# danieleschmidt/spin-glass-anneal-rl

Measured on AMD Instinct MI355X. Metric: spin-flip attempts/s (replicas x spins x sweeps / s), higher is better.
Workload: dtype f32

## Files before the change

spin-glass-anneal-rl_amd/csrc/sweep_dense_rs.hip:

```cpp
#include <cstdio>
#include <cstring>
#include <type_traits>

#include "sweep_common.h"

namespace sga {

template <bool GRID>
using RsPlanArg = typename std::conditional<GRID, RowSharedGridPlan, RowSharedPlan>::type;
__device__ __forceinline__ const RowSharedPlan &rs_plan(const RowSharedPlan &p) { return p; }
__device__ __forceinline__ const RowSharedPlan &rs_plan(const RowSharedGridPlan &g) { return g.p; }
__device__ __forceinline__ int rs_grid_k(const RowSharedPlan &) { return 0; }
__device__ __forceinline__ int rs_grid_k(const RowSharedGridPlan &g) { return g.k; }

__device__ __forceinline__ void rs_bit_of(int j, int &w32, unsigned int &bit) {
    const int g = j >> 8, e = j & 255, l = e >> 2, q = e & 3;
    w32 = 2 * (4 * g + q) + (l >> 5);
    bit = 1u << (l & 31);
}

__device__ __forceinline__ void rs_update(const SweepArgs &a, int r, int k, int t, int &site, uint32_t &ubits) {
    const u32x4 w = philox4x32_10((uint32_t)(t >> 1), a.sweep0 + (uint32_t)k, a.replica0 + (uint32_t)r, DOMAIN_SWEEP,
                                  a.seed_lo, a.seed_hi);
    const bool second = t & 1;
// ... 186 lines not shown
    for (int j = 0; j < NP; ++j) {
        const int x = tid + j * T, rr = x >> lhalf, b = x & hmask;
#pragma unroll
        for (int h = 0; h < 2; ++h) {
            const int s = site[2 * j + h];
            if (s < 0) continue;
            int ls;
            const int tl = rs_tile_of(s, S, mul, ls) - tl0;
            stage[atomicAdd(&cnt[(tl << log_trg) + rr], 1)] = ls | (rr << 12) | ((2 * b + h) << 17);
        }
    }
    __syncthreads();
    int *dst = p.ent + (long long)a.R * t0 + (long long)r0 * nt + below;
    for (int i = tid, m = sums[1]; i < m; i += T) dst[i] = stage[i];
}

template <typename JE, int PL, bool GRID>
__device__ __forceinline__ int rs_row_to_planes(const JE *row, int n, unsigned long long *planes, int lane, int wv, int gk) {
    const int nseg = (n + 255) >> 8, nw = 4 * nseg;
    int absum = 0;
    for (int g0 = wv; g0 < nseg; g0 += 16) {
        int v[4][4];
#pragma unroll
        for (int s = 0; s < 4; ++s) {
            const int e = 256 * (g0 + 4 * s) + 4 * lane;
            if (g0 + 4 * s < nseg && e < n) {
                if constexpr (std::is_same<JE, float>::value) {
                    float4 x = *reinterpret_cast<const float4 *>(row + e);
                    if constexpr (GRID) x.x = ldexpf(x.x, gk), x.y = ldexpf(x.y, gk), x.z = ldexpf(x.z, gk), x.w = ldexpf(x.w, gk);
                    v[s][0] = (int)x.x, v[s][1] = (int)x.y, v[s][2] = (int)x.z, v[s][3] = (int)x.w;
                } else {
                    const int x = *reinterpret_cast<const int *>(row + e);
#pragma unroll
                    for (int q = 0; q < 4; ++q) v[s][q] = (int)(int8_t)(x >> (8 * q));
                }
            } else {
#pragma unroll
                for (int q = 0; q < 4; ++q) v[s][q] = 0;
            }
#pragma unroll
            for (int q = 0; q < 4; ++q)
                if (e + q >= n) v[s][q] = 0;
        }
#pragma unroll
        for (int s = 0; s < 4; ++s) {
            const int g = g0 + 4 * s;
            if (g >= nseg) break;
#pragma unroll
            for (int q = 0; q < 4; ++q) {
                const int m = v[s][q] < 0 ? -v[s][q] : v[s][q];
                absum += m;
                const unsigned long long sg = ballot64(v[s][q] < 0);
                unsigned long long pb[PL];
#pragma unroll
                for (int b = 0; b < PL; ++b) pb[b] = ballot64(((m >> b) & 1) != 0);
                if (lane == 0) {
                    planes[4 * g + q] = sg;
#pragma unroll
                    for (int b = 0; b < PL; ++b) planes[(long long)(1 + b) * nw + 4 * g + q] = pb[b];
                }
            }
        }
    }
    return absum;
}

template <typename JE, int PL>
__global__ void __launch_bounds__(256) rs_planes_kernel(const JE *J, long long ldj, int n, unsigned long long *jp, int *jabs) {
    __shared__ int csum[4];
    const int i = blockIdx.x, lane = threadIdx.x & 63, wv = threadIdx.x >> 6;
    const int nw = 4 * ((n + 255) >> 8);
    int absum = rs_row_to_planes<JE, PL, false>(J + (long long)i * ldj, n, jp + (long long)i * (PL + 1) * nw, lane, wv, 0);
    absum = wave_sum(absum);
    if (lane == 0) csum[wv] = absum;
    __syncthreads();
    if (threadIdx.x == 0) jabs[i] = csum[0] + csum[1] + csum[2] + csum[3];
}
template <int PL>
__global__ void __launch_bounds__(256) rs_planes_grid_kernel(const float *J, long long ldj, int n, unsigned long long *jp, int *jabs,
                                                             int gk) {
    __shared__ int csum[4];
    const int i = blockIdx.x, lane = threadIdx.x & 63, wv = threadIdx.x >> 6;
    const int nw = 4 * ((n + 255) >> 8);
    int absum = rs_row_to_planes<float, PL, true>(J + (long long)i * ldj, n, jp + (long long)i * (PL + 1) * nw, lane, wv, gk);
    absum = wave_sum(absum);
    if (lane == 0) csum[wv] = absum;
    __syncthreads();
    if (threadIdx.x == 0) jabs[i] = csum[0] + csum[1] + csum[2] + csum[3];
}

template <int PL>
__global__ void __launch_bounds__(256) rs_fields_planes_kernel(const SweepArgs a, RowSharedPlan p, int win) {
    const int i = blockIdx.x, n = a.n;
    const int *off = p.off + (long long)win * (n + 1);
    const int lo = off[i], hi = off[i + 1];
    if (lo == hi) return;
    extern __shared__ ulonglong2 prow[];
    const int nw2 = p.nw32 >> 2;
    const int tid = threadIdx.x, lane = tid & 63, wv = tid >> 6, sub = lane >> 4, l16 = lane & 15;
    const ulonglong2 *src = reinterpret_cast<const ulonglong2 *>(p.jp) + (long long)i * (PL + 1) * nw2;
    for (int c = tid; c < (PL + 1) * nw2; c += 256) prow[c] = src[c];
    const int C = p.jabs[i];
    __syncthreads();
    const ulonglong2 *bits = reinterpret_cast<const ulonglong2 *>(p.bits);
    const int wmask = (1 << p.log_w) - 1;
    for (int x0 = lo + 4 * wv; x0 < hi; x0 += 16) {
        const int x = x0 + sub;
        const bool live = x < hi;
        const int e = p.ent[live ? x : lo];
        const ulonglong2 *s = bits + (long long)(e >> p.log_w) * nw2;
        int acc = 0;
        for (int c = l16; c < nw2; c += 16) {
            const ulonglong2 sv = s[c], sg = prow[c];
            const unsigned long long x0w = sv.x ^ sg.x, x1w = sv.y ^ sg.y;
#pragma unroll
            for (int b = 0; b < PL; ++b) {
                const ulonglong2 pb = prow[(1 + b) * nw2 + c];
                acc += (__popcll(pb.x & x0w) + __popcll(pb.y & x1w)) << b;
            }
        }
        acc += dpp_move<DPP_QUAD_XOR1>(acc);
        acc += dpp_move<DPP_QUAD_XOR2>(acc);
        acc += dpp_move<DPP_ROW_HALF_MIRROR>(acc);
        acc += dpp_move<DPP_ROW_MIRROR>(acc);
        if (live && l16 == 0) p.base[(long long)(e >> p.log_w) * p.W + (e & wmask)] = C - 2 * acc;
    }
}

template <int PL, bool ONES>
__device__ __forceinline__ int rs_tile_word(const ulonglong2 sv, const ulonglong2 *row, int nw2, int c) {
    const ulonglong2 sg = row[c];
    const unsigned long long x0w = sv.x ^ sg.x, x1w = sv.y ^ sg.y;
    if constexpr (ONES) {
        return __popcll(x0w) + __popcll(x1w);
    } else {
        int acc = 0;
#pragma unroll
        for (int b = 0; b < PL; ++b) {
            const ulonglong2 pb = row[(1 + b) * nw2 + c];
            acc += (__popcll(pb.x & x0w) + __popcll(pb.y & x1w)) << b;
        }
        return acc;
    }
}

struct RsTileChunk {
    const int *sent;
    const unsigned short *sls;
    const int *sjabs;
    const ulonglong2 *prow, *bits;
    int *base;
    int cn, nw2, rw2, log_w, W, nwaves;
};
template <int PL, bool ONES, int NK>
__device__ __forceinline__ void rs_tile_pieces(const RsTileChunk &ch, int wv, int sub, int l16) {
    const int L = (ch.cn + 4 * ch.nwaves - 1) / (4 * ch.nwaves), x1 = (4 * wv + sub) * L, wmask = (1 << ch.log_w) - 1;
    constexpr int NR = NK > 0 ? NK : 1;
    const int clast = l16 + 16 * (NR - 1);
    const bool vlast = clast < ch.nw2;
    const int cl = vlast ? clast : 0;
    ulonglong2 sv[NR];
#pragma unroll
    for (int k = 0; k < NR; ++k) sv[k] = make_ulonglong2(0ull, 0ull);
    int rcur = -1;
    for (int t = 0; t < L; ++t) {
        const int x = x1 + t;
        const bool live = x < ch.cn;
        const int e = ch.sent[live ? x : 0], lsd = ch.sls[live ? x : 0], ls = lsd & 0x7fff, r = e >> ch.log_w;
        const ulonglong2 *s = ch.bits + (long long)r * ch.nw2;
        const ulonglong2 *row = ch.prow + ls * ch.rw2;
        int acc = 0;
        if constexpr (NK > 0) {
            if (live && r != rcur) {
                rcur = r;
#pragma unroll
                for (int k = 0; k < NK - 1; ++k) sv[k] = s[l16 + 16 * k];
                sv[NK - 1] = s[cl];
            }
#pragma unroll
            for (int k = 0; k < NK - 1; ++k) acc += rs_tile_word<PL, ONES>(sv[k], row, ch.nw2, l16 + 16 * k);
            const int last = rs_tile_word<PL, ONES>(sv[NK - 1], row, ch.nw2, cl);
            acc += vlast ? last : 0;
        } else {
            for (int c = l16; c < ch.nw2; c += 16) acc += rs_tile_word<PL, ONES>(s[c], row, ch.nw2, c);
        }
        acc += dpp_move<DPP_QUAD_XOR1>(acc);
        acc += dpp_move<DPP_QUAD_XOR2>(acc);
        acc += dpp_move<DPP_ROW_HALF_MIRROR>(acc);
        acc += dpp_move<DPP_ROW_MIRROR>(acc);
        if (live && l16 == 0) ch.base[(long long)r * ch.W + (e & wmask)] = ch.sjabs[ls] - 2 * (acc - (lsd >> 15));
    }
}

template <int PL, bool ONES>
__global__ void __launch_bounds__(RS_TILE_THREADS) rs_fields_tiles_kernel(const SweepArgs a, RowSharedPlan p, int S, int log_trg,
                                                                         int win) {
    constexpr int RP = ONES ? 1 : PL + 1, T = RS_TILE_THREADS, NW = T / 64;
    const int n = a.n, R = a.R, tile0 = blockIdx.x * S, ns = min(S, n - tile0);
    extern __shared__ ulonglong2 prow[];
    const int nw2 = p.nw32 >> 2, rw2 = RP * nw2;
    int *sent = reinterpret_cast<int *>(prow + (size_t)S * rw2);
    int *spre = sent + RS_TILE_ENTRIES;
    int *sjabs = spre + R + S + 1;
    int *wtot = sjabs + S;
    unsigned short *sls = reinterpret_cast<unsigned short *>(wtot + NW);
    const int tid = threadIdx.x, lane = tid & 63, wv = __builtin_amdgcn_readfirstlane(tid >> 6), sub = lane >> 4, l16 = lane & 15;
    const int nsl = (R + (1 << log_trg) - 1) >> log_trg, t0 = win << p.log_w, nt = min(p.W, n - t0);
    const bool last = blockIdx.x + 1 == gridDim.x;
    const unsigned short *run0 = reinterpret_cast<const unsigned short *>(p.cnt) + ((long long)win * gridDim.x + blockIdx.x) * nsl;
    const unsigned short *run1 = run0 + nsl;
    int total;
    {
        const int per = (nsl + T - 1) / T, s0 = tid * per;
        int sum = 0;
        for (int j = 0; j < per; ++j)
            if (s0 + j < nsl) sum += (last ? min(1 << log_trg, R - ((s0 + j) << log_trg)) * nt : (int)run1[s0 + j]) - (int)run0[s0 + j];
        int inc = sum;
#pragma unroll
        for (int d = 1; d < 64; d <<= 1) {
            const int t = __shfl_up(inc, d);
            if (lane >= d) inc += t;
        }
        if (lane == 63) wtot[wv] = inc;
        __syncthreads();
        int run = inc - sum;
        total = 0;
        for (int w = 0; w < NW; ++w) {
            if (w < wv) run += wtot[w];
            total += wtot[w];
        }
        if (total == 0) return;
        for (int j = 0; j < per; ++j)
            if (s0 + j < nsl) {
                spre[s0 + j] = run;
                run += (last ? min(1 << log_trg, R - ((s0 + j) << log_trg)) * nt : (int)run1[s0 + j]) - (int)run0[s0 + j];
            }
    }
    for (int s = tid; s < ns; s += T) sjabs[s] = p.jabs[tile0 + s];
    for (int s = wv; s < ns; s += NW) {
        const ulonglong2 *src = reinterpret_cast<const ulonglong2 *>(p.jp) + (long long)(tile0 + s) * (PL + 1) * nw2;
        for (int c = lane; c < rw2; c += 64) prow[s * rw2 + c] = src[c];
    }
    const ulonglong2 *bits = reinterpret_cast<const ulonglong2 *>(p.bits);
    const int *went = p.ent + (long long)R * t0;
    for (int c0 = 0; c0 < total; c0 += RS_TILE_ENTRIES) {
        const int cn = min(RS_TILE_ENTRIES, total - c0);
        __syncthreads();
        for (int sb = wv; sb < nsl; sb += 64 * NW) {
            const int sm = sb + NW * lane;
            int st = 0, b0 = 0, b1 = 0;
            if (sm < nsl) st = run0[sm], b0 = spre[sm], b1 = sm + 1 < nsl ? spre[sm + 1] : total;
            const int nrun = min(64, (nsl - sb + NW - 1) / NW);
            for (int i = 0; i < nrun; ++i) {
                const int B0 = read_lane(b0, i), x0 = max(B0, c0), x1 = min(read_lane(b1, i), c0 + cn);
                if (x0 >= x1) continue;
                const int rs0 = (sb + NW * i) << log_trg;
                const int *src = went + (long long)rs0 * nt + read_lane(st, i) - B0;
                for (int g = x0 + lane; g < x1; g += 64) {
                    const int v = src[g], r = rs0 + ((v >> 12) & 31);
                    int ls = v & 0xfff;
                    if constexpr (ONES) {
                        int w32;
                        unsigned int bit;
                        rs_bit_of(tile0 + ls, w32, bit);
                        if (p.bits[(long long)r * p.nw32 + w32] & bit) ls |= 0x8000;
                    }
                    sent[g - c0] = (r << p.log_w) | (v >> 17);
                    sls[g - c0] = (unsigned short)ls;
                }
            }
        }
        __syncthreads();
        const RsTileChunk ch{sent, sls, sjabs, prow, bits, p.base, cn, nw2, rw2, p.log_w, p.W, NW};
        constexpr int NKMAX = row_shared_tile_register_words(PL);
        const int nk = (nw2 + 15) >> 4;
        switch (nk <= NKMAX ? nk : 0) {
            case 1: rs_tile_pieces<PL, ONES, NKMAX >= 1 ? 1 : 0>(ch, wv, sub, l16); break;
            case 2: rs_tile_pieces<PL, ONES, NKMAX >= 2 ? 2 : 0>(ch, wv, sub, l16); break;
            case 3: rs_tile_pieces<PL, ONES, NKMAX >= 3 ? 3 : 0>(ch, wv, sub, l16); break;
            case 4: rs_tile_pieces<PL, ONES, NKMAX >= 4 ? 4 : 0>(ch, wv, sub, l16); break;
            case 5: rs_tile_pieces<PL, ONES, NKMAX >= 5 ? 5 : 0>(ch, wv, sub, l16); break;
            case 6: rs_tile_pieces<PL, ONES, NKMAX >= 6 ? 6 : 0>(ch, wv, sub, l16); break;
            case 7: rs_tile_pieces<PL, ONES, NKMAX >= 7 ? 7 : 0>(ch, wv, sub, l16); break;
            case 8: rs_tile_pieces<PL, ONES, NKMAX >= 8 ? 8 : 0>(ch, wv, sub, l16); break;
            default: rs_tile_pieces<PL, ONES, 0>(ch, wv, sub, l16); break;
        }
    }
}

template <typename JE, int PL, bool GRID>
__global__ void __launch_bounds__(256) rs_fields_kernel(const SweepArgs a, const RsPlanArg<GRID> pg, int win) {
    const RowSharedPlan &p = rs_plan(pg);
    const int i = blockIdx.x, n = a.n;
    const int *off = p.off + (long long)win * (n + 1);
    const int lo = off[i], hi = off[i + 1];
    if (lo == hi) return;
    extern __shared__ unsigned long long planes[];
    __shared__ int csum[4];
    const int nseg = (n + 255) >> 8, nw = 4 * nseg;
    const int tid = threadIdx.x, lane = tid & 63, wv = tid >> 6;
    const JE *row = reinterpret_cast<const JE *>(a.J) + (long long)i * a.ldj;
    int absum = rs_row_to_planes<JE, PL, GRID>(row, n, planes, lane, wv, rs_grid_k(pg));
    absum = wave_sum(absum);
    if (lane == 0) csum[wv] = absum;
    __syncthreads();
    const int C = csum[0] + csum[1] + csum[2] + csum[3];
    const unsigned long long *bits = reinterpret_cast<const unsigned long long *>(p.bits);
    const int wmask = (1 << p.log_w) - 1;
    for (int x = lo + wv; x < hi; x += 8) {
        const bool two = x + 4 < hi;
        const int e0 = p.ent[x], e1 = two ? p.ent[x + 4] : e0;
        const unsigned long long *s0 = bits + (long long)(e0 >> p.log_w) * nw;
        const unsigned long long *s1 = bits + (long long)(e1 >> p.log_w) * nw;
        int acc0 = 0, acc1 = 0;
        for (int c = lane; c < nw; c += 64) {
            const unsigned long long sg = planes[c];
            const unsigned long long x0 = s0[c] ^ sg, x1 = s1[c] ^ sg;
#pragma unroll
            for (int b = 0; b < PL; ++b) {
                const unsigned long long pb = planes[(long long)(1 + b) * nw + c];
                acc0 += __popcll(pb & x0) << b;
                acc1 += __popcll(pb & x1) << b;
            }
        }
        wave_sum2(acc0, acc1);
        if (lane == 0) {
            p.base[(long long)(e0 >> p.log_w) * p.W + (e0 & wmask)] = C - 2 * acc0;
            if (two) p.base[(long long)(e1 >> p.log_w) * p.W + (e1 & wmask)] = C - 2 * acc1;
        }
    }
}

__device__ __forceinline__ bool rs_accept(float fk, float u, double T, int table_m) {
    if (fk <= 0.0f) return true;
    if (fk <= (float)table_m) return u < expf_det((float)(-(double)(2 * (int)fk) / T));
    const double dE = (double)(2.0f * fk);
    return (dE > T * 104.0) ? false : (u < expf_det((float)(-dE / T)));
}

template <typename JE, bool BITS, bool ONES = false>
struct RsRaw {
    typename std::conditional<BITS, typename std::conditional<ONES, uint32_t, uint2>::type, JE>::type v;
};
template <typename JE, bool BITS, bool ONES>
__device__ __forceinline__ void rs_coupling_load(RsRaw<JE, BITS, ONES> &raw, const SweepArgs &a, const RowSharedPlan &p, int sa,
                                                 unsigned int voff) {
    if constexpr (BITS && ONES) {
        const char *sgn = reinterpret_cast<const char *>(p.jp) + (long long)sa * (8ll * p.nw32);
        raw.v = *reinterpret_cast<const uint32_t *>(sgn + voff);
    } else if constexpr (BITS) {
        const char *sgn = reinterpret_cast<const char *>(p.jp) + (long long)sa * (8ll * p.nw32);
        const char *mag = sgn + 4ll * p.nw32;
        raw.v = make_uint2(*reinterpret_cast<const uint32_t *>(sgn + voff), *reinterpret_cast<const uint32_t *>(mag + voff));
    } else {
        const char *row = reinterpret_cast<const char *>(a.J) + (long long)sa * a.ldj * (long long)sizeof(JE);
        raw.v = *reinterpret_cast<const JE *>(row + voff);
    }
}
template <typename JE, bool BITS>
__device__ __forceinline__ float rs_coupling(const RsRaw<JE, BITS> &raw, unsigned int bit, float unit) {
    if constexpr (BITS) return (raw.v.y & bit) ? ((raw.v.x & bit) ? -unit : unit) : 0.0f;
    else return (float)raw.v;
}
template <typename JE>
__device__ __forceinline__ float rs_coupling(const RsRaw<JE, true, true> &raw, unsigned int bit, float unit, bool same) {
    return same ? 0.0f : ((raw.v & bit) ? -unit : unit);
}

#ifndef SGA_RS_CHAIN_PRIO
#define SGA_RS_CHAIN_PRIO 3
#endif
constexpr int RS_CHAIN_PRIO = SGA_RS_CHAIN_PRIO;
constexpr int RS_CHAIN_K = 4;
constexpr int RS_CHAIN_U = 8;
#ifndef SGA_RS_CHAIN_TABLE
#define SGA_RS_CHAIN_TABLE 1
#endif
constexpr bool RS_CHAIN_TABLE = SGA_RS_CHAIN_TABLE != 0;
#ifndef SGA_RS_CHAIN_STAGED
#define SGA_RS_CHAIN_STAGED 1
#endif
constexpr bool RS_CHAIN_STAGED = SGA_RS_CHAIN_STAGED != 0;
#ifndef SGA_RS_CHAIN_INDEXED
#define SGA_RS_CHAIN_INDEXED 1
#endif
constexpr bool RS_CHAIN_INDEXED = SGA_RS_CHAIN_INDEXED != 0;

template <typename T, int NB>
struct RsBlockRegs {
#if SGA_RS_CHAIN_INDEXED
    typedef T V __attribute__((ext_vector_type(NB)));
    V v;
#else
    T v[NB];
#endif
};

__device__ __forceinline__ bool rs_accept_tabled(const float *ptab, int Q, bool zero_tail, float fk, float u, double T, int table_m) {
    if (fk <= 0.0f) return true;
    const int q = (int)fk;
    if (q <= Q) return u < ptab[q];
    if (zero_tail) return false;
    return rs_accept(fk, u, T, table_m);
}

template <bool GRID>
__device__ __forceinline__ bool rs_decide(int cs, float cf, float chh, float cu, double T, int table_m) {
    if constexpr (GRID) {
        double dE;
        return metropolis_accept(SGA_RULE_METROPOLIS, SGA_ARITH_F64, cf, cs, chh, 0.0f, T, cu, dE);
    } else {
        return rs_accept((float)cs * (cf + chh), cu, T, table_m);
    }
}
template <bool GRID, bool ANYRULE>
__device__ __forceinline__ bool rs_decide_rule(int rule, int cs, float cf, float chh, float cu, double T, int table_m) {
    if constexpr (ANYRULE) {
        double dE;
        return metropolis_accept(rule, SGA_ARITH_F64, cf, cs, chh, 0.0f, T, cu, dE);
    } else {
        return rs_decide<GRID>(cs, cf, chh, cu, T, table_m);
// ... 172 lines not shown
    if (ones) return planes == 1 ? reinterpret_cast<const void *>(rs_fields_tiles_kernel<1, true>) : nullptr;
    switch (planes) {
        case 1: return reinterpret_cast<const void *>(rs_fields_tiles_kernel<1, false>);
        case 3: return reinterpret_cast<const void *>(rs_fields_tiles_kernel<3, false>);
        case 8: return reinterpret_cast<const void *>(rs_fields_tiles_kernel<8, false>);
        default: return nullptr;
    }
}
hipError_t row_shared_tiles_prepare(int planes, bool ones, size_t lds_bytes) {
    const void *kern = rs_tiles_kernel_of(planes, ones);
    if (!kern || lds_bytes > RS_TILE_LDS_BUDGET) return hipErrorInvalidValue;
    return ensure_lds_limit(kern, lds_bytes);
}
template <typename Kern>
static hipError_t rs_launch_tiles(Kern kern, const SweepArgs &a, const RowSharedPlan &p, const RowSharedTiles &t, int log_trg,
                                  int win, hipStream_t st) {
    const size_t lds = row_shared_tile_lds(a.n, p.planes, t.ones != 0, t.S, a.R);
    hipError_t e = ensure_lds_limit(reinterpret_cast<const void *>(kern), lds);
    if (e != hipSuccess) return e;
    hipLaunchKernelGGL(kern, dim3((a.n + t.S - 1) / t.S), dim3(RS_TILE_THREADS), lds, st, a, p, t.S, log_trg, win);
    return hipGetLastError();
}
static hipError_t rs_fields_tiles(const SweepArgs &a, const RowSharedPlan &p, const RowSharedTiles &t, int log_trg, int win,
                                  hipStream_t st) {
    if (t.ones) return rs_launch_tiles(rs_fields_tiles_kernel<1, true>, a, p, t, log_trg, win, st);
    switch (p.planes) {
        case 1: return rs_launch_tiles(rs_fields_tiles_kernel<1, false>, a, p, t, log_trg, win, st);
        case 3: return rs_launch_tiles(rs_fields_tiles_kernel<3, false>, a, p, t, log_trg, win, st);
        case 8: return rs_launch_tiles(rs_fields_tiles_kernel<8, false>, a, p, t, log_trg, win, st);
        default: return hipErrorInvalidValue;
    }
}

template <typename JE>
static hipError_t rs_fields(const SweepArgs &a, const RowSharedPlan &p, int grid, const RowSharedTiles &tiles, int log_trg, int win,
                            hipStream_t st) {
    const size_t lds = (size_t)(p.planes + 1) * (p.nw32 / 2) * 8;
    if (p.jp && tiles.S > 0) return rs_fields_tiles(a, p, tiles, log_trg, win, st);
    if (p.jp) {
        switch (p.planes) {
            case 1: return rs_launch_fields(rs_fields_planes_kernel<1>, lds, a, p, win, st);
            case 3: return rs_launch_fields(rs_fields_planes_kernel<3>, lds, a, p, win, st);
            case 8: return rs_launch_fields(rs_fields_planes_kernel<8>, lds, a, p, win, st);
            default: return hipErrorInvalidValue;
        }
    }
    if constexpr (std::is_same<JE, float>::value) {
        if (grid > 1) {
            const RowSharedGridPlan g{p, grid - 1};
            switch (p.planes) {
                case 1: return rs_launch_fields(rs_fields_kernel<JE, 1, true>, lds, a, g, win, st);
                case 3: return rs_launch_fields(rs_fields_kernel<JE, 3, true>, lds, a, g, win, st);
                case 8: return rs_launch_fields(rs_fields_kernel<JE, 8, true>, lds, a, g, win, st);
                default: return hipErrorInvalidValue;
            }
        }
    }
    switch (p.planes) {
        case 1: return rs_launch_fields(rs_fields_kernel<JE, 1, false>, lds, a, p, win, st);
        case 3: return rs_launch_fields(rs_fields_kernel<JE, 3, false>, lds, a, p, win, st);
        case 8: return rs_launch_fields(rs_fields_kernel<JE, 8, false>, lds, a, p, win, st);
        default: return hipErrorInvalidValue;
    }
}

template <typename JE, bool BITS, bool GRID, bool ANYRULE, bool ONES>
static hipError_t rs_chain_launch(const SweepArgs &a, const RsPlanArg<GRID> &p, int W, int k, int win, hipStream_t st) {
    switch (W) {
        case 256: hipLaunchKernelGGL((rs_chain_kernel<JE, 4, BITS, GRID, ANYRULE, ONES>), dim3(a.R), dim3(64), 0, st, a, p, k, win); break;
        case 512: hipLaunchKernelGGL((rs_chain_kernel<JE, 8, BITS, GRID, ANYRULE, ONES>), dim3(a.R), dim3(64), 0, st, a, p, k, win); break;
        case 1024: hipLaunchKernelGGL((rs_chain_kernel<JE, 16, BITS, GRID, ANYRULE, ONES>), dim3(a.R), dim3(64), 0, st, a, p, k, win); break;
        default: return hipErrorInvalidValue;
    }
    return hipGetLastError();
}
template <typename JE, bool BITS, bool ONES = false>
static hipError_t rs_chain(const SweepArgs &a, const RowSharedPlan &p, int grid, int k, int win, hipStream_t st) {
    if (a.rule != SGA_RULE_METROPOLIS) {
        if (grid) return rs_chain_launch<JE, BITS, true, true, ONES>(a, RowSharedGridPlan{p, grid - 1}, p.W, k, win, st);
        return rs_chain_launch<JE, BITS, false, true, ONES>(a, p, p.W, k, win, st);
    }
    if (grid) return rs_chain_launch<JE, BITS, true, false, ONES>(a, RowSharedGridPlan{p, grid - 1}, p.W, k, win, st);
    return rs_chain_launch<JE, BITS, false, false, ONES>(a, p, p.W, k, win, st);
}

template <typename JE>
static hipError_t rs_build_planes(const void *J, long long ldj, int n, int planes, unsigned long long *jp, int *jabs,
                                  hipStream_t st) {
    const JE *Jt = reinterpret_cast<const JE *>(J);
    switch (planes) {
        case 1: hipLaunchKernelGGL((rs_planes_kernel<JE, 1>), dim3(n), dim3(256), 0, st, Jt, ldj, n, jp, jabs); break;
        case 3: hipLaunchKernelGGL((rs_planes_kernel<JE, 3>), dim3(n), dim3(256), 0, st, Jt, ldj, n, jp, jabs); break;
        case 8: hipLaunchKernelGGL((rs_planes_kernel<JE, 8>), dim3(n), dim3(256), 0, st, Jt, ldj, n, jp, jabs); break;
        default: return hipErrorInvalidValue;
    }
    return hipGetLastError();
}
static hipError_t rs_build_planes_grid(const void *J, long long ldj, int n, int planes, int gk, unsigned long long *jp, int *jabs,
                                       hipStream_t st) {
    const float *Jt = reinterpret_cast<const float *>(J);
    switch (planes) {
        case 1: hipLaunchKernelGGL((rs_planes_grid_kernel<1>), dim3(n), dim3(256), 0, st, Jt, ldj, n, jp, jabs, gk); break;
        case 3: hipLaunchKernelGGL((rs_planes_grid_kernel<3>), dim3(n), dim3(256), 0, st, Jt, ldj, n, jp, jabs, gk); break;
        case 8: hipLaunchKernelGGL((rs_planes_grid_kernel<8>), dim3(n), dim3(256), 0, st, Jt, ldj, n, jp, jabs, gk); break;
        default: return hipErrorInvalidValue;
    }
    return hipGetLastError();
}

hipError_t launch_rs_build_planes(const void *J, bool j_is_i8, long long ldj, int n, int planes, int grid_k,
                                  unsigned long long *jp, int *jabs, hipStream_t st) {
    if (!J || !jp || !jabs || n <= 0 || grid_k < 0 || grid_k > 30 || (j_is_i8 && grid_k != 0)) return hipErrorInvalidValue;
    if (j_is_i8) return rs_build_planes<int8_t>(J, ldj, n, planes, jp, jabs, st);
    return grid_k ? rs_build_planes_grid(J, ldj, n, planes, grid_k, jp, jabs, st)
                  : rs_build_planes<float>(J, ldj, n, planes, jp, jabs, st);
}

struct RsGroupLaunch {
    SweepArgs a;
    RowSharedPlan p;
    hipStream_t st = nullptr;
    RowSharedTilePlan tp;
    size_t tlds = 0;
    int log_trg = 0;
    dim3 pgrid, tgrid;
};

static void rs_group_args(const SweepArgs &a, const RowSharedPlan &p, const RowSharedGroups &g, int i, SweepArgs &ag, RowSharedPlan &pg) {
    const int r0 = g.begin[i];
    const RowSharedGroupView v = row_shared_group_view(a.n, p.W, g, i);
    ag = a;
    ag.R = g.begin[i + 1] - r0;
    ag.replica0 = a.replica0 + (uint32_t)r0;
    ag.spins = a.spins + (long long)r0 * a.sstride;
    ag.energy = a.energy + r0;
    ag.best_energy = a.best_energy ? a.best_energy + r0 : nullptr;
    ag.best_spins = a.best_spins ? a.best_spins + (long long)r0 * a.sstride : nullptr;
    ag.n_accepted = a.n_accepted + r0;
    ag.rep_temp = a.rep_temp ? a.rep_temp + r0 : nullptr;
    ag.sched = a.sched ? a.sched + (long long)r0 * a.sched_rs : nullptr;
    pg = p;
    pg.cnt = p.cnt + v.cnt;
    pg.ent = p.ent + v.ent;
    pg.base = p.base + v.base;
    pg.bits = p.bits + v.bits;
    pg.n_groups = v.n_groups;
}

hipError_t launch_sweep_dense_rs(const SweepArgs &a, const RowSharedPlan &p, bool j_is_i8, hipStream_t st, int grid,
                                 RowSharedTiles tiles, const RowSharedGroupRun *run) {
    if (tiles.S > 0 && (!p.jp || tiles.S > RS_TILE_MAX_SITES || a.R > RS_TILE_MAX_REPLICAS || (tiles.ones && p.planes != 1) ||
                        row_shared_tile_lds(a.n, p.planes, tiles.ones != 0, tiles.S, a.R) > RS_TILE_LDS_BUDGET))
        return hipErrorInvalidValue;
    if (a.reps_per_model < 0 || (a.reps_per_model > 0 && a.model_stride_j != 0)) return hipErrorInvalidValue;
    if (a.rep_list || a.R <= 0 || a.n <= 0 || (p.W != 256 && p.W != 512 && p.W != 1024) || (1 << p.log_w) != p.W)
        return hipErrorInvalidValue;
    if (p.log_rg < 0 || p.n_groups != (a.R + (1 << p.log_rg) - 1) >> p.log_rg || (p.jp && !p.jabs) || !p.tot)
        return hipErrorInvalidValue;
    if (grid < 0 || grid > 31 || (j_is_i8 && grid > 1)) return hipErrorInvalidValue;
    if (a.rule != SGA_RULE_METROPOLIS && a.rule != SGA_RULE_GLAUBER && a.rule != SGA_RULE_HEAT_BATH) return hipErrorInvalidValue;
    if (a.rule != SGA_RULE_METROPOLIS && a.arith != SGA_ARITH_F64) return hipErrorInvalidValue;
    const int nwin = (a.n + p.W - 1) / p.W;
    const size_t plds = sizeof(int) * (size_t)(a.n < RS_PLAN_TILE ? a.n : RS_PLAN_TILE);
    const dim3 sgrid(row_shared_scan_chunks(a.n), nwin);
    const bool chain_bits = p.jp && p.planes == 1;
    const bool by_tile = p.jp && tiles.S > 0;
    const bool chain_ones = chain_bits && by_tile && tiles.ones;
    const int ntiles = by_tile ? (a.n + tiles.S - 1) / tiles.S : 0;
    const RowSharedGroups groups = row_shared_groups(a.R, run ? run->G : 1);
    const int G = groups.G;
    if (run && run->G > 1 && (G != run->G || !by_tile || a.energy_trace || !run->fork || !row_shared_groups_fit(a.n, p.W, tiles.S, a.R, groups)))
        return hipErrorInvalidValue;
    RsGroupLaunch gl[RS_MAX_GROUPS];
    for (int g = 0; g < G; ++g) {
        RsGroupLaunch &q = gl[g];
        if (G > 1) {
            rs_group_args(a, p, groups, g, q.a, q.p);
            q.st = g ? run->stream[g - 1] : st;
            if (g && (!q.st || !run->join[g - 1])) return hipErrorInvalidValue;
        } else {
            q.a = a, q.p = p, q.st = st;
        }
        q.pgrid = dim3(q.p.n_groups, nwin, (a.n + RS_PLAN_TILE - 1) / RS_PLAN_TILE);
        if (by_tile) {
            q.tp = row_shared_tile_plan(a.n, p.W, tiles.S, q.a.R);
            if (q.tp.rg <= 0) return hipErrorInvalidValue;
            while ((1 << q.log_trg) < q.tp.rg) ++q.log_trg;
            q.tlds = row_shared_tile_plan_lds(p.W, q.tp.rg, q.tp.tiles);
            const hipError_t le = ensure_lds_limit(reinterpret_cast<const void *>(rs_tile_plan_kernel), q.tlds);
            if (le != hipSuccess) return le;
        }
        q.tgrid = dim3(by_tile ? (q.a.R + q.tp.rg - 1) / q.tp.rg : 1, nwin, by_tile ? (ntiles + q.tp.tiles - 1) / q.tp.tiles : 1);
    }
    hipError_t e = hipSuccess;
    if (G > 1) {
        e = hipEventRecord(run->fork, st);
        for (int g = 1; g < G && e == hipSuccess; ++g) e = hipStreamWaitEvent(gl[g].st, run->fork, 0);
        if (e != hipSuccess) return e;
    }
    for (int g = 0; g < G && e == hipSuccess; ++g) {
        hipLaunchKernelGGL(rs_pack_kernel, dim3(gl[g].a.R), dim3(256), 0, gl[g].st, gl[g].a, gl[g].p);
        e = hipGetLastError();
    }
    for (int k = 0; k < a.n_sweeps && e == hipSuccess; ++k) {
        for (int g = 0; g < G && e == hipSuccess; ++g) {
            const RsGroupLaunch &q = gl[g];
            if (by_tile) {
                hipLaunchKernelGGL(rs_tile_plan_kernel, q.tgrid, dim3(RS_TILE_PLAN_THREADS), q.tlds, q.st, q.a, q.p, k, tiles.S, q.log_trg,
                                   q.tp.tiles);
            } else {
                hipLaunchKernelGGL(rs_plan_kernel<false>, q.pgrid, dim3(256), plds, q.st, q.a, q.p, k);
                hipLaunchKernelGGL(rs_scan_totals_kernel, sgrid, dim3(RS_SCAN_CHUNK), 0, q.st, q.a, q.p);
                hipLaunchKernelGGL(rs_scan_kernel, sgrid, dim3(RS_SCAN_CHUNK), 0, q.st, q.a, q.p);
                hipLaunchKernelGGL(rs_plan_kernel<true>, q.pgrid, dim3(256), plds, q.st, q.a, q.p, k);
            }
            e = hipGetLastError();
        }
        for (int w = 0; w < nwin && e == hipSuccess; ++w) {
            for (int g = 0; g < G && e == hipSuccess; ++g) {
                const RsGroupLaunch &q = gl[g];
                e = j_is_i8 ? rs_fields<int8_t>(q.a, q.p, grid, tiles, q.log_trg, w, q.st)
                            : rs_fields<float>(q.a, q.p, grid, tiles, q.log_trg, w, q.st);
                if (e != hipSuccess) break;
                if (chain_ones)
                    e = j_is_i8 ? rs_chain<int8_t, true, true>(q.a, q.p, grid, k, w, q.st) : rs_chain<float, true, true>(q.a, q.p, grid, k, w, q.st);
                else if (chain_bits)
                    e = j_is_i8 ? rs_chain<int8_t, true>(q.a, q.p, grid, k, w, q.st) : rs_chain<float, true>(q.a, q.p, grid, k, w, q.st);
                else
                    e = j_is_i8 ? rs_chain<int8_t, false>(q.a, q.p, grid, k, w, q.st) : rs_chain<float, false>(q.a, q.p, grid, k, w, q.st);
            }
        }
        for (int g = 0; g < G && e == hipSuccess && !a.no_best; ++g) {
            const RsGroupLaunch &q = gl[g];
            e = launch_update_best(q.a.energy, q.a.spins, q.a.best_energy, q.a.best_spins, q.a.sstride, q.a.R, q.st);
        }
    }
    if (G > 1) {
        hipError_t je = hipSuccess;
        for (int g = 1; g < G; ++g) {
            hipError_t x = hipEventRecord(run->join[g - 1], gl[g].st);
            if (x == hipSuccess) x = hipStreamWaitEvent(st, run->join[g - 1], 0);
            if (x != hipSuccess) (void)hipStreamSynchronize(gl[g].st), je = x;
        }
        if (e == hipSuccess) e = je;
    }
    if (e == hipSuccess) {
        char gs[48] = "", ts[64] = "", rg[24] = "";
        if (grid) std::snprintf(gs, sizeof(gs), ", grid=2^-%d", grid - 1);
        if (a.rule != SGA_RULE_METROPOLIS)
            std::snprintf(gs + std::strlen(gs), sizeof(gs) - std::strlen(gs), ", rule=%s", a.rule == SGA_RULE_GLAUBER ? "glauber" : "heat-bath");
        if (p.jp && tiles.S > 0) std::snprintf(ts, sizeof(ts), " in tiles of %d sites%s", tiles.S, tiles.ones ? ", sign-only" : "");
        if (G > 1) std::snprintf(rg, sizeof(rg), " groups=%d", G);
        note_sweep_kernel("sweep_dense_rs<%s, planes=%d, W=%d%s> (row-shared windows: plan, fields from %s%s, chain)%s",
                          j_is_i8 ? "int8_t" : "float", p.planes, p.W, gs, p.jp ? "resident bit-planes" : "on-chip conversion", ts, rg);
    }
    return e;
}

}
```

Before: 11.95 billion.

## Prefetch tile rows and flatten entry gather in fields-tiles kernel prologue

The fields-tiles kernel now issues its global loads for the tile's J-rows and jabs into registers before the replica-run prefix scan, then writes them to LDS afterwards, so load latency overlaps the scan. Entry gathering is reworked: each thread binary-searches the prefix array to locate its entry's run, replacing the per-wave serial loop over runs. The inner tile loop is also made leaner, prefetching the next entry, using 24-bit multiplies and byte offsets. This costs more registers per thread and adds a launch check that bounds offsets so 32-bit arithmetic stays valid.

Result: faster. 12.51 billion (median of 6 runs) (+4.7%).

```diff
diff --git a/profiles/fields_prologue_timing.py b/profiles/fields_prologue_timing.py
--- /dev/null
+++ b/profiles/fields_prologue_timing.py
@@ -0,0 +1,244 @@
+import argparse
+import csv
+import glob
+import json
+import os
+import subprocess
+import sys
+import tempfile
+import time
+
+import numpy as np
+
+ROOT = os.path.dirname(os.path.dirname(os.path.abspath(__file__)))
+OUT = os.path.join(ROOT, "profiles", "fields_prologue.json")
+COUNTERS = ["SQ_WAVE_CYCLES", "SQ_WAIT_ANY", "SQ_INSTS_VALU", "SQ_ACTIVE_INST_VALU", "SQ_INSTS_LDS"]
+WARMUP, STEPS, N = 5, 20, 10000
+FIT_R = (128, 256, 512, 1024)
+
+
+def last_json(text):
+    return json.loads(next(ln for ln in text.splitlines()[::-1] if ln.startswith("{")))
+
+
+def env_of(lib):
+    env = dict(os.environ)
+    env["SGA_LIBRARY_PATH"] = os.path.abspath(lib)
+    return env
+
+
+def step_on_device(cmd, env, limit=300, cwd=None):
+    p = subprocess.run(["timeout", "-k", "10", str(limit)] + cmd, env=env, capture_output=True, text=True, cwd=cwd)
+    if p.returncode != 0:
+        raise SystemExit(f"{cmd}: exit {p.returncode} -- stopping here\n{p.stderr[-800:]}")
+    return p.stdout
+
+
+def drive(R, G, W, kind):
+    sys.path.insert(0, ROOT)
+    import spin_glass_anneal_rl_amd as sg
+    rng = np.random.RandomState(7)
+    if kind == "tern":
+        A = rng.randint(-1, 2, (N, N), dtype=np.int8) * (rng.randint(0, 100, (N, N), dtype=np.int8) < 45)
+    elif kind == "a7":
+        A = rng.randint(-7, 8, (N, N), dtype=np.int8)
+    else:
+        A = rng.randint(0, 2, (N, N), dtype=np.int8) * 2 - 1
+    A = np.triu(A.astype(np.int8), 1)
+    J = (A + A.T).astype(np.float32) * np.float32(0.25 if kind == "grid" else 1.0)
+    hi, lo = (2.5, 0.025) if kind == "grid" else (10.0, 0.1)
+    with sg.AnnealEngine(0) as e:
+        if kind != "tune":
+            e.set_option("row_shared", 1)
+            e.set_option("row_shared_window", W)
+            e.set_option("row_shared_grid", 1 if kind == "grid" else 0)
+            e.set_replica_groups(G)
+        if kind in ("tern", "a7"):
+            e.set_option("row_shared_fields", 1)
+        e.set_tuning(sweeps_per_launch=1)
+        if kind == "glauber":
+            e.set_update_rule(sg._native.RULE_GLAUBER)
+        e.set_dense(J, np.zeros(N, np.float32), storage="f32")
+        e.init_replicas(R, seed=11)
+        e.set_ladder(np.asarray([hi * (lo / hi) ** (i / max(R - 1, 1)) for i in range(R)]))
+        if kind == "tune":
+            ms = e.autotune()
+            e.sweep(1)
+            print(json.dumps({"autotune_ms": ms, "table": {str(k): v for k, v in e.autotune_table(forms=True).items()},
+                              "kernel": e.last_kernel()}, default=str))
+            return
+        done = 0
+
+        def step():
+            nonlocal done
+            e.sweep(1)
+            done += 1
+            if done % 10 == 0:
+                e.exchange(count=False)
+        for _ in range(WARMUP):
+            step()
+        e.energies()
+        e.enable_timing(True)
+        e.kernel_time(reset=True)
+        t0 = time.perf_counter()
+        for _ in range(STEPS):
+            step()
+        e.energies()
+        wall = time.perf_counter() - t0
+        launches, kernel_ms = e.kernel_time(reset=True)
+        print(json.dumps({"R": R, "G": G, "W": W, "kind": kind, "ms_per_step_wall": wall * 1e3 / STEPS,
+                          "ms_per_sweep_events": kernel_ms / max(launches, 1), "kernel": e.last_kernel(),
+                          "checksum": float(np.asarray(e.energies()).sum())}))
+
+
+def drive_cmd(R, G, W=1024, kind="c2a"):
+    return [sys.executable, os.path.abspath(__file__), "--drive", str(R), str(G), str(W), kind]
+
+
+def profiled(cmd, env, rocprof_args, pattern):
+    with tempfile.TemporaryDirectory() as d:
+        out = step_on_device(["rocprofv3"] + rocprof_args + ["-d", d, "--output-format", "csv", "--"] + cmd, env, limit=500)
+        table = list(csv.reader(open(glob.glob(os.path.join(d, "**", pattern), recursive=True)[0])))
+    return last_json(out), table
+
+
+def trace_cell(lib, R, G):
+    res, trace = profiled(drive_cmd(R, G), env_of(lib), ["--kernel-trace", "--stats"], "*kernel_trace.csv")
+    col = {h: i for i, h in enumerate(trace[0])}
+    rows = sorted(((int(r[col["Start_Timestamp"]]), int(r[col["End_Timestamp"]]), r[col["Kernel_Name"]])
+                   for r in trace[1:] if "sga::rs_" in r[col["Kernel_Name"]]), key=lambda x: x[0])
+    out = {"ms_per_sweep_events": res["ms_per_sweep_events"], "kernel": res["kernel"]}
+    for part in ("rs_chain_kernel", "rs_fields_tiles_kernel"):
+        mine = [r for r in rows if "sga::" + part in r[2]]
+        us = np.asarray([(b - a) / 1e3 for a, b, _ in mine[WARMUP * len(mine) // (WARMUP + STEPS):]])
+        out[part] = {"launches": len(us), "avg_us": float(us.mean()), "min_us": float(us.min()), "max_us": float(us.max())}
+    return out
+
+
+def pmc_cell(lib, G):
+    _, rows = profiled(drive_cmd(1024, G), env_of(lib), ["--pmc"] + COUNTERS, "*counter_collection.csv")
+    col = {h: i for i, h in enumerate(rows[0])}
+    disp = {}
+    for r in rows[1:]:
+        if "sga::rs_fields_tiles_kernel" in r[col["Kernel_Name"]]:
+            disp.setdefault(int(r[col["Dispatch_Id"]]), {})[r[col["Counter_Name"]]] = float(r[col["Counter_Value"]])
+    ids = sorted(disp)
+    ids = ids[WARMUP * len(ids) // (WARMUP + STEPS):]
+    tot = {c + "_per_launch": sum(disp[i].get(c, 0.0) for i in ids) / len(ids) for c in COUNTERS}
+    tot["dispatches"] = len(ids)
+    tot["wait_any_share"] = tot["SQ_WAIT_ANY_per_launch"] / tot["SQ_WAVE_CYCLES_per_launch"]
+    return tot
+
+
+def bench(lib, extra, dump=None):
+    cmd = [sys.executable, os.path.join(ROOT, "bench.py"), "--gpus", "1"] + list(extra) + (["--dump-outputs", dump] if dump else [])
+    res = last_json(step_on_device(cmd, env_of(lib), limit=600, cwd=ROOT))
+    return res["ms_per_step"], res.get("roofline", {}).get("kernel_instantiation")
+
+
+def headline(base, mine):
+    spread = max(base) - min(base)
+    return {"parent_spread_ms": spread, "parent_fastest_minus_new_slowest_ms": min(base) - max(mine),
+            "wins": bool(min(base) - max(mine) > 0 and min(base) - max(mine) >= 3 * spread)}
+
+
+def main():
+    ap = argparse.ArgumentParser()
+    ap.add_argument("--parts", default="ab,trace,pmc,fit,cells,by")
+    ap.add_argument("--runs", type=int, default=5)
+    ap.add_argument("--cell-runs", type=int, default=3)
+    ap.add_argument("--variants", default="")
+    ap.add_argument("--profile-variants", default="", help="the libraries of trace, pmc and fit (default: all)")
+    ap.add_argument("--drive", nargs=4, help=argparse.SUPPRESS)
+    a = ap.parse_args()
+    if a.drive:
+        return drive(int(a.drive[0]), int(a.drive[1]), int(a.drive[2]), a.drive[3])
+    libs = dict(v.split("=") for v in a.variants.split(",") if v)
+    pair = {k: libs[k] for k in ("parent", "new")}
+    merged = json.load(open(OUT)) if os.path.exists(OUT) else {}
+
+    def save():
+        json.dump(merged, open(OUT, "w"), indent=1)
+
+    def cells(shapes, which, into):
+        for R, G, W, kind in shapes:
+            key = f"R{R}_G{G}_W{W}_{kind}"
+            cell = merged.setdefault(into, {}).setdefault(key, {})
+            for _ in range(a.cell_runs):
+                for name, lib in which.items():
+                    res = last_json(step_on_device(drive_cmd(R, G, W, kind), env_of(lib)))
+                    c = cell.setdefault(name, {"events_ms": [], "wall_ms": []})
+                    c["events_ms"].append(res["ms_per_sweep_events"])
+                    c["wall_ms"].append(res["ms_per_step_wall"])
+                    c.update(kernel=res["kernel"], checksum=res["checksum"])
+                    print(into, key, name, res["ms_per_sweep_events"], flush=True)
+                    save()
+            for name in which:
+                cell[name]["median_events_ms"] = float(np.median(cell[name]["events_ms"]))
+                cell[name]["same_checksum_as_parent"] = cell[name]["checksum"] == cell["parent"]["checksum"]
+            save()
+
+    parts = a.parts.split(",")
+    ab = merged.setdefault("ab_c2a", {})
+    for tag, extra, runs in (("steps50_warmup10", ["--steps", "50", "--warmup", "10"], a.runs), ("default", [], 3)):
+        if "ab" in parts or "ab:" + tag in parts:
+            ms, kern = {t: [] for t in pair}, {}
+            for _ in range(runs):
+                for t in pair:
+                    v, kern[t] = bench(pair[t], extra)
+                    ms[t].append(v)
+                    print("ab", tag, t, v, flush=True)
+            ab[tag] = dict(headline(ms["parent"], ms["new"]), ms_per_step=ms, kernel=kern)
+            save()
+    if "ab" in parts or "ab:dump" in parts:
+        with tempfile.TemporaryDirectory() as d:
+            for t in pair:
+                bench(pair[t], ["--steps", "20", "--warmup", "5"], dump=os.path.join(d, t))
+            names = sorted(os.listdir(os.path.join(d, "parent")))
+            same = names == sorted(os.listdir(os.path.join(d, "new"))) and all(
+                np.array_equal(np.load(os.path.join(d, "parent", f)), np.load(os.path.join(d, "new", f))) for f in names)
+        ab.update(dumped_arrays=names, dumped_arrays_equal=bool(same))
+        print("ab", json.dumps(ab), flush=True)
+        save()
+    prof = {k: libs[k] for k in a.profile_variants.split(",") if k} or libs
+    if "trace" in parts:
+        for name, lib in prof.items():
+            merged.setdefault("trace_c2a_W1024_G2", {})[name] = trace_cell(lib, 1024, 2)
+            print("trace", name, json.dumps(merged["trace_c2a_W1024_G2"][name]), flush=True)
+            save()
+    if "pmc" in parts:
+        for name, lib in prof.items():
+            merged.setdefault("pmc_tiles_c2a_W1024_G2", {})[name] = pmc_cell(lib, 2)
+            print("pmc", name, json.dumps(merged["pmc_tiles_c2a_W1024_G2"][name]), flush=True)
+            save()
+    if "fit" in parts:
+        for name, lib in prof.items():
+            us = [trace_cell(lib, R, 1)["rs_fields_tiles_kernel"]["avg_us"] for R in FIT_R]
+            b, a0 = np.polyfit(np.asarray(FIT_R, float), np.asarray(us), 1)
+            merged.setdefault("fit_fields_G1_W1024", {})[name] = {"replicas": list(FIT_R), "avg_us": us, "intercept_us": float(a0),
+                                                                  "us_per_replica": float(b)}
+            print("fit", name, json.dumps(merged["fit_fields_G1_W1024"][name]), flush=True)
+            save()
+    if "cells" in parts:
+        cells([(1024, 2, 1024, "c2a"), (1024, 1, 1024, "c2a")], libs, "cells")
+    if "by" in parts or "by:cells" in parts:
+        cells([(1024, 2, 512, "c2a"), (1024, 2, 256, "c2a"), (256, 2, 1024, "c2a"), (1024, 2, 1024, "glauber"), (1024, 2, 1024, "grid"),
+               (1024, 2, 1024, "tern"), (1024, 2, 1024, "a7")], pair, "bystanders")
+    if "by" in parts or "by:other" in parts:
+        for wl in ("c3", "c4", "c5"):
+            ms = {t: [] for t in pair}
+            for _ in range(3):
+                for t in pair:
+                    ms[t].append(bench(pair[t], ["--workload", wl])[0])
+            merged.setdefault("other_workloads", {})[wl] = {"ms_per_step": ms, "median": {k: float(np.median(v)) for k, v in ms.items()}}
+            print(wl, json.dumps(merged["other_workloads"][wl]), flush=True)
+            save()
+    if "by" in parts or "by:tune" in parts:
+        for t in pair:
+            merged.setdefault("autotune_c2a", {})[t] = last_json(step_on_device(drive_cmd(1024, 0, 0, "tune"), env_of(pair[t]), limit=500))
+            print("tune", t, json.dumps(merged["autotune_c2a"][t]), flush=True)
+            save()
+
+
+if __name__ == "__main__":
+    main()
diff --git a/spin-glass-anneal-rl_amd/csrc/sweep_dense_rs.hip b/spin-glass-anneal-rl_amd/csrc/sweep_dense_rs.hip
--- a/spin-glass-anneal-rl_amd/csrc/sweep_dense_rs.hip
+++ b/spin-glass-anneal-rl_amd/csrc/sweep_dense_rs.hip
@@ -362,6 +362,15 @@
     int *base;
     int cn, nw2, rw2, log_w, W, nwaves;
 };
+#ifndef SGA_RS_TILES_LEAN
+#define SGA_RS_TILES_LEAN 1
+#endif
+constexpr bool RS_TILES_LEAN = SGA_RS_TILES_LEAN != 0;
+#ifndef SGA_RS_TILES_PROLOGUE
+#define SGA_RS_TILES_PROLOGUE 1
+#endif
+constexpr bool RS_TILES_PROLOGUE = SGA_RS_TILES_PROLOGUE != 0;
+
 template <int PL, bool ONES, int NK>
 __device__ __forceinline__ void rs_tile_pieces(const RsTileChunk &ch, int wv, int sub, int l16) {
     const int L = (ch.cn + 4 * ch.nwaves - 1) / (4 * ch.nwaves), x1 = (4 * wv + sub) * L, wmask = (1 << ch.log_w) - 1;
@@ -373,6 +382,49 @@
 #pragma unroll
     for (int k = 0; k < NR; ++k) sv[k] = make_ulonglong2(0ull, 0ull);
     int rcur = -1;
+    if constexpr (RS_TILES_LEAN) {
+        const char *bitsb = reinterpret_cast<const char *>(ch.bits), *prowb = reinterpret_cast<const char *>(ch.prow);
+        char *baseb = reinterpret_cast<char *>(ch.base);
+        const unsigned int rowb = 16u * (unsigned int)ch.nw2, lrowb = 16u * (unsigned int)ch.rw2;
+        const unsigned int o16 = 16u * (unsigned int)l16, ocl = 16u * (unsigned int)cl;
+        bool live_n = x1 < ch.cn;
+        unsigned int e_n = (unsigned int)ch.sent[live_n ? x1 : 0], lsd_n = ch.sls[live_n ? x1 : 0];
+        for (int t = 0; t < L; ++t) {
+            const bool live = live_n;
+            const unsigned int e = e_n, lsd = lsd_n, ls = lsd & 0x7fffu;
+            const int xn = x1 + t + 1;
+            live_n = xn < ch.cn;
+            e_n = (unsigned int)ch.sent[live_n ? xn : 0], lsd_n = ch.sls[live_n ? xn : 0];
+            const int r = (int)(e >> ch.log_w);
+            const unsigned int bo = __umul24((unsigned int)r, rowb);
+            const ulonglong2 *row = reinterpret_cast<const ulonglong2 *>(prowb + __umul24(ls, lrowb));
+            int acc = 0;
+            if constexpr (NK > 0) {
+                if (live && r != rcur) {
+                    rcur = r;
+                    const char *s = bitsb + (size_t)(bo + o16);
+#pragma unroll
+                    for (int k = 0; k < NK - 1; ++k) sv[k] = *reinterpret_cast<const ulonglong2 *>(s + 256 * k);
+                    sv[NK - 1] = *reinterpret_cast<const ulonglong2 *>(bitsb + (size_t)(bo + ocl));
+                }
+#pragma unroll
+                for (int k = 0; k < NK - 1; ++k) acc += rs_tile_word<PL, ONES>(sv[k], row, ch.nw2, l16 + 16 * k);
+                const int last = rs_tile_word<PL, ONES>(sv[NK - 1], row, ch.nw2, cl);
+                acc += vlast ? last : 0;
+            } else {
+                for (int c = l16; c < ch.nw2; c += 16)
+                    acc += rs_tile_word<PL, ONES>(*reinterpret_cast<const ulonglong2 *>(bitsb + (size_t)(bo + 16u * (unsigned int)c)), row,
+                                                  ch.nw2, c);
+            }
+            acc += dpp_move<DPP_QUAD_XOR1>(acc);
+            acc += dpp_move<DPP_QUAD_XOR2>(acc);
+            acc += dpp_move<DPP_ROW_HALF_MIRROR>(acc);
+            acc += dpp_move<DPP_ROW_MIRROR>(acc);
+            if (live && l16 == 0)
+                *reinterpret_cast<int *>(baseb + (size_t)(e << 2)) = ch.sjabs[ls] - 2 * (acc - (int)(lsd >> 15));
+        }
+        return;
+    }
     for (int t = 0; t < L; ++t) {
         const int x = x1 + t;
         const bool live = x < ch.cn;
@@ -420,11 +472,52 @@
     const unsigned short *run0 = reinterpret_cast<const unsigned short *>(p.cnt) + ((long long)win * gridDim.x + blockIdx.x) * nsl;
     const unsigned short *run1 = run0 + nsl;
     int total;
+    constexpr int NJB = RS_TILE_MAX_SITES / T;
+    constexpr int NPW = (int)((RS_TILE_LDS_BUDGET - 6 * RS_TILE_ENTRIES) / 16 + T - 1) / T;
+    constexpr int NEN = RS_TILE_ENTRIES / T;
+    const int npw = ns * rw2;
+    const bool have_sd = 2 * nsl <= R + S + 1;
+    int *sd = spre + nsl;
+    int st1 = 0, jb[NJB], li[NPW];
+    ulonglong2 pw[NPW];
     {
         const int per = (nsl + T - 1) / T, s0 = tid * per;
         int sum = 0;
-        for (int j = 0; j < per; ++j)
-            if (s0 + j < nsl) sum += (last ? min(1 << log_trg, R - ((s0 + j) << log_trg)) * nt : (int)run1[s0 + j]) - (int)run0[s0 + j];
+        int en1 = 0;
+        if (RS_TILES_PROLOGUE && per == 1) {
+            const unsigned short *end1 = last ? run0 : run1;
+            const int s1 = min(tid, nsl - 1);
+            st1 = run0[s1];
+            en1 = end1[s1];
+        }
+        if constexpr (RS_TILES_PROLOGUE) {
+#pragma unroll
+            for (int j = 0; j < NJB; ++j) {
+                jb[j] = 0;
+                if (j * T < ns) jb[j] = p.jabs[tile0 + min(tid + j * T, ns - 1)];
+            }
+            const ulonglong2 *jp2 = reinterpret_cast<const ulonglong2 *>(p.jp) + (long long)tile0 * (PL + 1) * nw2;
+            const unsigned int mul = 0xffffffffu / (unsigned int)rw2 + 1u;
+#pragma unroll
+            for (int j = 0; j < NPW; ++j) {
+                pw[j] = make_ulonglong2(0ull, 0ull);
+                li[j] = -1;
+                if (j * T < npw) {
+                    const int c = tid + j * T;
+                    int col;
+                    const int s = rs_tile_of(min(c, npw - 1), rw2, mul, col);
+                    pw[j] = jp2[(long long)s * ((PL + 1) * nw2) + col];
+                    li[j] = c < npw ? c : -1;
+                }
+            }
+        }
+        if (RS_TILES_PROLOGUE && per == 1) {
+            const int len = (last ? min(1 << log_trg, R - (tid << log_trg)) * nt : en1) - st1;
+            sum = tid < nsl ? len : 0;
+        } else {
+            for (int j = 0; j < per; ++j)
+                if (s0 + j < nsl) sum += (last ? min(1 << log_trg, R - ((s0 + j) << log_trg)) * nt : (int)run1[s0 + j]) - (int)run0[s0 + j];
+        }
         int inc = sum;
 #pragma unroll
         for (int d = 1; d < 64; d <<= 1) {
@@ -440,43 +533,112 @@
             total += wtot[w];
         }
         if (total == 0) return;
-        for (int j = 0; j < per; ++j)
-            if (s0 + j < nsl) {
-                spre[s0 + j] = run;
-                run += (last ? min(1 << log_trg, R - ((s0 + j) << log_trg)) * nt : (int)run1[s0 + j]) - (int)run0[s0 + j];
-            }
-    }
-    for (int s = tid; s < ns; s += T) sjabs[s] = p.jabs[tile0 + s];
-    for (int s = wv; s < ns; s += NW) {
-        const ulonglong2 *src = reinterpret_cast<const ulonglong2 *>(p.jp) + (long long)(tile0 + s) * (PL + 1) * nw2;
-        for (int c = lane; c < rw2; c += 64) prow[s * rw2 + c] = src[c];
+        if (RS_TILES_PROLOGUE && per == 1) {
+            if (tid < nsl) {
+                spre[tid] = run;
+                if (have_sd) sd[tid] = st1 - run;
+            }
+        } else {
+            for (int j = 0; j < per; ++j)
+                if (s0 + j < nsl) {
+                    const int b = run0[s0 + j];
+                    spre[s0 + j] = run;
+                    if (RS_TILES_PROLOGUE && have_sd) sd[s0 + j] = b - run;
+                    run += (last ? min(1 << log_trg, R - ((s0 + j) << log_trg)) * nt : (int)run1[s0 + j]) - b;
+                }
+        }
+    }
+    if constexpr (RS_TILES_PROLOGUE) {
+#pragma unroll
+        for (int j = 0; j < NJB; ++j)
+            if (j * T < ns && tid + j * T < ns) sjabs[tid + j * T] = jb[j];
+#pragma unroll
+        for (int j = 0; j < NPW; ++j)
+            if (j * T < npw && li[j] >= 0) prow[li[j]] = pw[j];
+    } else {
+        for (int s = tid; s < ns; s += T) sjabs[s] = p.jabs[tile0 + s];
+        for (int s = wv; s < ns; s += NW) {
+            const ulonglong2 *src = reinterpret_cast<const ulonglong2 *>(p.jp) + (long long)(tile0 + s) * (PL + 1) * nw2;
+            for (int c = lane; c < rw2; c += 64) prow[s * rw2 + c] = src[c];
+        }
     }
     const ulonglong2 *bits = reinterpret_cast<const ulonglong2 *>(p.bits);
     const int *went = p.ent + (long long)R * t0;
+    const int btop = nsl > 1 ? 1 << (31 - __clz(nsl - 1)) : 0;
     for (int c0 = 0; c0 < total; c0 += RS_TILE_ENTRIES) {
         const int cn = min(RS_TILE_ENTRIES, total - c0);
         __syncthreads();
-        for (int sb = wv; sb < nsl; sb += 64 * NW) {
-            const int sm = sb + NW * lane;
-            int st = 0, b0 = 0, b1 = 0;
-            if (sm < nsl) st = run0[sm], b0 = spre[sm], b1 = sm + 1 < nsl ? spre[sm + 1] : total;
-            const int nrun = min(64, (nsl - sb + NW - 1) / NW);
-            for (int i = 0; i < nrun; ++i) {
-                const int B0 = read_lane(b0, i), x0 = max(B0, c0), x1 = min(read_lane(b1, i), c0 + cn);
-                if (x0 >= x1) continue;
-                const int rs0 = (sb + NW * i) << log_trg;
-                const int *src = went + (long long)rs0 * nt + read_lane(st, i) - B0;
-                for (int g = x0 + lane; g < x1; g += 64) {
-                    const int v = src[g], r = rs0 + ((v >> 12) & 31);
-                    int ls = v & 0xfff;
+        if constexpr (RS_TILES_PROLOGUE) {
+            int g[NEN], sl[NEN], v[NEN];
+            unsigned int ob[NEN];
+#pragma unroll
+            for (int j = 0; j < NEN; ++j) g[j] = min(c0 + tid + j * T, c0 + cn - 1), sl[j] = 0;
+            for (int b = btop; b; b >>= 1) {
+#pragma unroll
+                for (int j = 0; j < NEN; ++j) {
+                    const int m = sl[j] + b;
+                    if (spre[min(m, nsl - 1)] <= g[j] && m < nsl) sl[j] = m;
+                }
+            }
+            const int w0 = c0 + 64 * wv;
+#pragma unroll
+            for (int j = 0; j < NEN; ++j) {
+                v[j] = 0;
+                if (w0 + j * T < c0 + cn) {
+                    const int d = have_sd ? sd[sl[j]] : (int)run0[sl[j]] - spre[sl[j]];
+                    v[j] = went[((sl[j] << log_trg) * nt + d) + g[j]];
+                }
+            }
+            if constexpr (ONES) {
+#pragma unroll
+                for (int j = 0; j < NEN; ++j) {
+                    ob[j] = 0u;
+                    if (w0 + j * T < c0 + cn) {
+                        int w32;
+                        unsigned int bit;
+                        rs_bit_of(tile0 + (v[j] & 0xfff), w32, bit);
+                        const int r = (sl[j] << log_trg) + ((v[j] >> 12) & 31);
+                        ob[j] = p.bits[(long long)r * p.nw32 + w32];
+                    }
+                }
+            }
+#pragma unroll
+            for (int j = 0; j < NEN; ++j)
+                if (w0 + j * T < c0 + cn && c0 + tid + j * T < c0 + cn) {
+                    const int r = (sl[j] << log_trg) + ((v[j] >> 12) & 31);
+                    int ls = v[j] & 0xfff;
                     if constexpr (ONES) {
                         int w32;
                         unsigned int bit;
                         rs_bit_of(tile0 + ls, w32, bit);
-                        if (p.bits[(long long)r * p.nw32 + w32] & bit) ls |= 0x8000;
+                        if (ob[j] & bit) ls |= 0x8000;
                     }
-                    sent[g - c0] = (r << p.log_w) | (v >> 17);
-                    sls[g - c0] = (unsigned short)ls;
+                    sent[tid + j * T] = (r << p.log_w) | (v[j] >> 17);
+                    sls[tid + j * T] = (unsigned short)ls;
+                }
+        } else {
+            for (int sb = wv; sb < nsl; sb += 64 * NW) {
+                const int sm = sb + NW * lane;
+                int st = 0, b0 = 0, b1 = 0;
+                if (sm < nsl) st = run0[sm], b0 = spre[sm], b1 = sm + 1 < nsl ? spre[sm + 1] : total;
+                const int nrun = min(64, (nsl - sb + NW - 1) / NW);
+                for (int i = 0; i < nrun; ++i) {
+                    const int B0 = read_lane(b0, i), x0 = max(B0, c0), x1 = min(read_lane(b1, i), c0 + cn);
+                    if (x0 >= x1) continue;
+                    const int rs0 = (sb + NW * i) << log_trg;
+                    const int *src = went + (long long)rs0 * nt + read_lane(st, i) - B0;
+                    for (int g = x0 + lane; g < x1; g += 64) {
+                        const int v = src[g], r = rs0 + ((v >> 12) & 31);
+                        int ls = v & 0xfff;
+                        if constexpr (ONES) {
+                            int w32;
+                            unsigned int bit;
+                            rs_bit_of(tile0 + ls, w32, bit);
+                            if (p.bits[(long long)r * p.nw32 + w32] & bit) ls |= 0x8000;
+                        }
+                        sent[g - c0] = (r << p.log_w) | (v >> 17);
+                        sls[g - c0] = (unsigned short)ls;
+                    }
                 }
             }
         }
@@ -955,6 +1117,7 @@
     if (tiles.S > 0 && (!p.jp || tiles.S > RS_TILE_MAX_SITES || a.R > RS_TILE_MAX_REPLICAS || (tiles.ones && p.planes != 1) ||
                         row_shared_tile_lds(a.n, p.planes, tiles.ones != 0, tiles.S, a.R) > RS_TILE_LDS_BUDGET))
         return hipErrorInvalidValue;
+    if (tiles.S > 0 && (4ll * p.nw32 >= (1ll << 18) || 4ll * p.nw32 * a.R > (1ll << 30))) return hipErrorInvalidValue;
     if (a.reps_per_model < 0 || (a.reps_per_model > 0 && a.model_stride_j != 0)) return hipErrorInvalidValue;
     if (a.rep_list || a.R <= 0 || a.n <= 0 || (p.W != 256 && p.W != 512 && p.W != 1024) || (1 << p.log_w) != p.W)
         return hipErrorInvalidValue;
```
